# google-deepmind/mujoco_warp

Hardware: NVIDIA H100
Metric: env-steps/sec (whole box) on humanoid.xml at nworld=8192 per GPU (higher is better)
Workload: dtype f32

## Files before the change

### include/mjb200.h

```cpp
#ifndef MJB200_H
#define MJB200_H

#ifdef __cplusplus
extern "C" {
#endif

typedef struct mjbModel mjbModel;
typedef struct mjbData mjbData;

mjbModel* mjb_model_create(void);
void mjb_model_destroy(mjbModel* m);
int mjb_model_set_int(mjbModel* m, const char* name, int value);
int mjb_model_set_float(mjbModel* m, const char* name, float value);
int mjb_model_set_array(mjbModel* m, const char* name, const void* dev_ptr, int nbatch);
int mjb_model_set_array_batched(mjbModel* m, const char* name, const void* dev_ptr, int nbatch, int batch_stride);
int mjb_model_finalize(mjbModel* m);

mjbData* mjb_data_create(int nworld, int nconmax, int naconmax, int njmax, int njmax_pad, int nv_pad);
void mjb_data_destroy(mjbData* d);
int mjb_data_set_array(mjbData* d, const char* name, void* dev_ptr);
int mjb_data_set_int(mjbData* d, const char* name, int value);
int mjb_data_finalize(mjbData* d, const mjbModel* m);

int mjb_step(const mjbModel* m, mjbData* d, void* stream);
// ... 16 lines not shown
int mjb_rne(const mjbModel* m, mjbData* d, void* stream);
int mjb_solve_m(const mjbModel* m, mjbData* d, float* x, const float* y, void* stream);
int mjb_mul_m(const mjbModel* m, mjbData* d, float* res, const float* vec, void* stream);
int mjb_sensor_pos(const mjbModel* m, mjbData* d, void* stream);
int mjb_sensor_vel(const mjbModel* m, mjbData* d, void* stream);
int mjb_sensor_acc(const mjbModel* m, mjbData* d, void* stream);
int mjb_contact_force(const mjbModel* m, mjbData* d, const int* contact_ids, int n, int to_world_frame, float* force, void* stream);
int mjb_rays(const mjbModel* m, mjbData* d, const float* pnt, const float* vec, int nray, int pnt_nbatch, const int* geomgroup,
             int flg_static, const int* bodyexclude, float* dist, int* geomid, float* normal, void* stream);
int mjb_rungekutta4(const mjbModel* m, mjbData* d, void* stream);
int mjb_solve(const mjbModel* m, mjbData* d, void* stream);
int mjb_euler(const mjbModel* m, mjbData* d, void* stream);
int mjb_implicit(const mjbModel* m, mjbData* d, void* stream);
#define MJB_SET_CONST_FIXED 1
#define MJB_SET_CONST_0 2
#define MJB_SET_CONST_SPRING 4
int mjb_set_const(const mjbModel* m, mjbData* d, int parts, int restore, void* stream);
int mjb_ctrl_noise(const mjbModel* m, mjbData* d, const float* ctrl_center, int step, float noise_std, float noise_rate, void* stream);

int mjb_step_profile(const mjbModel* m, mjbData* d, void* stream, float* ms_out);

int mjb_team_residency(const mjbModel* m, const mjbData* d, int* position_worlds, int* velocity_worlds);

int mjb_last_launch_count(void);
const char* mjb_last_error(void);
const char* mjb_version(void);

#ifdef __cplusplus
}
#endif
#endif
```

### mujoco_warp_b200/__init__.py

```python

from . import scenes
from ._src import mjcf
from ._src._lib import build
from ._src.forward import camlight, collision, com_pos, crb, ctrl_noise, euler, factor_m, forward, fwd_acceleration, fwd_actuation
from ._src.forward import fwd_position, fwd_velocity, kinematics, last_launch_count, make_constraint, solve, step, step_profile, team_residency, transmission
from ._src.forward import com_vel, contact_force, fwd_kinematics, get_state, implicit, mul_m, passive, rne, rungekutta4, sensor_acc, sensor_pos, sensor_vel, set_state, solve_m, step1, step2
from ._src.inverse import inverse
from ._src.ray import ray, rays
from ._src.set_const import set_const, set_const_0, set_const_fixed, set_const_spring
from ._src.io import get_data_into, load_trajectory, make_data, override_model, put_data, put_model, reset_data, reset_data_keyframe
from ._src.trace import event_trace_step, flatten_trace
from ._src.types import BroadphaseFilter, BroadphaseType, ConeType, Constraint, ConstraintState, ConstraintType, Contact, Data
from ._src.types import BiasType, DynType, GainType, State, Statistic, TrnType
from ._src.types import DisableBit, EnableBit, GeomType, IntegratorType, JointType, Model, Option, OverflowType, SolverType

__all__ = [n for n in dir() if not n.startswith("_")]
```

### mujoco_warp_b200/_src/forward.py

```python

from __future__ import annotations

import torch

from . import _lib
from .types import Data, Model


def _call(name: str, m: Model, d: Data):
  if d._model is not m and d._model._handle != m._handle:
    raise ValueError("Data was created for a different Model")
  stream = torch.cuda.current_stream().cuda_stream
  _lib.check(getattr(_lib.lib(), name)(m._handle, d._handle, stream))


def step(m: Model, d: Data):
  _call("mjb_step", m, d)


def forward(m: Model, d: Data):
  _call("mjb_forward", m, d)


def fwd_position(m: Model, d: Data):
# ... 202 lines not shown
  return int(_lib.lib().mjb_last_launch_count())


KERNEL_NAMES = ("position", "collision", "constraint", "velocity", "solver", "integrate")


def step_profile(m: Model, d: Data):
  import ctypes

  out = (ctypes.c_float * 6)()
  stream = torch.cuda.current_stream().cuda_stream
  _lib.check(_lib.lib().mjb_step_profile(m._handle, d._handle, stream, out))
  return dict(zip(KERNEL_NAMES, [float(x) for x in out]))


def team_residency(m: Model, d: Data):
  import ctypes

  f = _lib.lib().mjb_team_residency
  f.argtypes = [ctypes.c_void_p, ctypes.c_void_p, ctypes.POINTER(ctypes.c_int), ctypes.POINTER(ctypes.c_int)]
  pos, vel = ctypes.c_int(), ctypes.c_int()
  _lib.check(f(m._handle, d._handle, ctypes.byref(pos), ctypes.byref(vel)))
  return {"position": pos.value, "velocity": vel.value}
```

### mujoco_warp_b200/csrc/capi.cu

```cuda
#include <cstdio>
#include <cstdlib>
#include <algorithm>
#include <cstring>
using std::min;
#include <string>

#include "../../include/mjb200.h"
#include "mjb_launch.cuh"
#include "mjb_types.cuh"

struct mjbModel {
  ModelDev dev;
  FluidDev fluid;
  SensorCollisionDev sc;
  SetConstDev setc;
  bool finalized;
};
struct mjbData {
  DataDev dev;
  bool finalized;
  cudaStream_t aux[8];
  cudaEvent_t ev_fork, ev_join[8];
  int nsplit;
  float* rk;
// ... 165 lines not shown
  if (check(cudaMemset(d->dev.world_ncon, 0, sizeof(int) * (size_t)d->dev.nworld), "memset")) return -1;
  if (check(cudaMalloc(&d->dev.imp_qacc, sizeof(float) * (size_t)d->dev.nworld * (size_t)(m->dev.nv > 0 ? m->dev.nv : 1)), "cudaMalloc(imp_qacc)")) return -1;
  if (!d->inv_qacc && check(cudaMalloc(&d->inv_qacc, sizeof(float) * (size_t)d->dev.nworld * (size_t)(m->dev.nv > 0 ? m->dev.nv : 1)), "cudaMalloc(inv_qacc)")) return -1;
  if (!d->qpos_save && check(cudaMalloc(&d->qpos_save, sizeof(float) * (size_t)d->dev.nworld * (size_t)(m->dev.nq > 0 ? m->dev.nq : 1)), "cudaMalloc(qpos_save)")) return -1;
  if (m->dev.integrator == INT_RK4 && !d->rk &&
      check(cudaMalloc(&d->rk, sizeof(float) * (size_t)d->dev.nworld * (size_t)(m->dev.nq + 3 * m->dev.nv + 2 * m->dev.na + 1)), "cudaMalloc(rk)")) return -1;
  const size_t smem[6] = {smem_position(m->dev, d->dev), smem_collision(m->dev, d->dev), smem_constraint(m->dev, d->dev),
                          smem_velocity(m->dev, d->dev, fluid(m, d)), smem_solver(m->dev, d->dev),    smem_integrate(m->dev)};
  static const char* names[6] = {"position", "collision", "constraint", "velocity", "solver", "integrate"};
  for (int i = 0; i < 6; i++)
    if (smem[i] > kMaxSmem) {
      char buf[160];
      snprintf(buf, sizeof buf, "%s kernel needs %zu B of shared memory per block (> %zu): model/njmax too large for this version", names[i], smem[i], kMaxSmem);
      return fail(buf);
    }
  if (smem_sensor_collision(m->sc) > kMaxSmem) {
    char buf[200];
    snprintf(buf, sizeof buf, "collision-sensor kernel needs %zu B of shared memory per block (> %zu): too many sensor geom pairs or GJK / EPA iterations",
             smem_sensor_collision(m->sc), kMaxSmem);
    return fail(buf);
  }
  {
    const char* e = getenv("MJB_SPLIT");
    const int want = e ? atoi(e) : 2;
    if (want >= 2 && d->dev.nworld >= 1024) {
      const int ns = want > 8 ? 8 : want;
      for (int i = 0; i < ns; i++) {
        if (check(cudaStreamCreateWithFlags(&d->aux[i], cudaStreamNonBlocking), "cudaStreamCreate")) return -1;
        if (check(cudaEventCreateWithFlags(&d->ev_join[i], cudaEventDisableTiming), "cudaEventCreate")) return -1;
      }
      if (check(cudaEventCreateWithFlags(&d->ev_fork, cudaEventDisableTiming), "cudaEventCreate")) return -1;
      d->nsplit = ns;
    }
  }
  d->finalized = true;
  return 0;
}

#define MJB_ENTER()                                                                 \
  if (!m || !d || !m->finalized || !d->finalized) return fail("model/data not finalized"); \
  cudaStream_t s = (cudaStream_t)stream;                                             \
  g_launches = 0;
#define MJB_LAUNCH(call) do { if (check((call), #call)) return -1; } while (0)

int mjb_kinematics(const mjbModel* m, mjbData* d, void* stream) { MJB_ENTER(); MJB_LAUNCH(launch_position(m->dev, d->dev, STG_KINEMATICS, s)); return 0; }
int mjb_com_pos(const mjbModel* m, mjbData* d, void* stream) { MJB_ENTER(); MJB_LAUNCH(launch_position(m->dev, d->dev, STG_COM_POS, s)); return 0; }
int mjb_camlight(const mjbModel* m, mjbData* d, void* stream) { MJB_ENTER(); MJB_LAUNCH(launch_position(m->dev, d->dev, STG_CAMLIGHT, s)); return 0; }
// ... 140 lines not shown
    return rk4_after_forward(m, d, s);
  }
  return pipeline(m, d, RUN_POSITION | RUN_VELOCITY | RUN_SOLVER | RUN_EULER, s);
}
int mjb_step_profile(const mjbModel* m, mjbData* d, void* stream, float* ms_out) {
  MJB_ENTER();
  cudaEvent_t ev[7];
  int n = 0, rc = 0;
  while (n < 7 && !(rc = check(cudaEventCreate(&ev[n]), "cudaEventCreate"))) n++;
  if (!rc) rc = check(reset_contact_counters(d->dev, s), "reset_contact_counters");
  if (!rc) rc = check(cudaEventRecord(ev[0], s), "cudaEventRecord");
  if (!rc) rc = chain(m, d, d->dev, RUN_POSITION | RUN_VELOCITY | RUN_SOLVER | RUN_EULER, s, ev + 1);
  if (!rc) rc = check(cudaEventSynchronize(ev[6]), "cudaEventSynchronize");
  for (int i = 0; i < 6 && !rc; i++) rc = check(cudaEventElapsedTime(&ms_out[i], ev[i], ev[i + 1]), "cudaEventElapsedTime");
  for (int i = 0; i < n; i++) cudaEventDestroy(ev[i]);
  return rc;
}
int mjb_team_residency(const mjbModel* m, const mjbData* d, int* position_worlds, int* velocity_worlds) {
  if (!m || !d || !m->finalized || !d->finalized) return fail("model/data not finalized");
  if (!position_worlds || !velocity_worlds) return fail("mjb_team_residency: null output");
  if (check(resident_worlds_position(m->dev, d->dev, position_worlds), "resident_worlds_position")) return -1;
  if (check(resident_worlds_velocity(m->dev, d->dev, velocity_worlds, fluid(m, d)), "resident_worlds_velocity")) return -1;
  return 0;
}
int mjb_set_const(const mjbModel* m, mjbData* d, int parts, int restore, void* stream) {
  MJB_ENTER();
  if (parts < 1 || parts > (MJB_SET_CONST_FIXED | MJB_SET_CONST_0 | MJB_SET_CONST_SPRING)) return fail("mjb_set_const: parts must be a non-empty combination of MJB_SET_CONST_FIXED / _0 / _SPRING, got " + std::to_string(parts));
  if (restore != 0 && restore != 1) return fail("mjb_set_const: restore must be 0 or 1");
  const ModelDev& md = m->dev;
  const int nworld = d->dev.nworld;
  const bool fixed = parts & MJB_SET_CONST_FIXED, zero = parts & MJB_SET_CONST_0, spring = (parts & MJB_SET_CONST_SPRING) && md.ntendon > 0;
  if (zero && (!m->setc.actuator_acc0 || !m->setc.meaninertia)) return fail("mjb_set_const: model array not set: actuator_acc0 / meaninertia");
  int w_zero = 1, w_spring = md.nb_tendon_lengthspring;
  struct { const char* name; int nb; } out[] = {
    {"body_subtreemass", fixed ? md.nb_body_subtreemass : 1}, {"tendon_lengthspring", spring ? md.nb_tendon_lengthspring : 1},
    {"tendon_length0", md.nb_tendon_length0}, {"eq_data", md.nb_eq_data}, {"dof_invweight0", md.nb_dof_invweight0}, {"body_invweight0", md.nb_body_invweight0},
    {"tendon_invweight0", md.nb_tendon_invweight0}, {"cam_pos0", md.nb_cam_pos0}, {"cam_poscom0", md.nb_cam_poscom0}, {"cam_mat0", md.nb_cam_mat0},
    {"light_pos0", md.nb_light_pos0}, {"light_poscom0", md.nb_light_poscom0}, {"light_dir0", md.nb_light_dir0}, {"actuator_acc0", m->setc.nb_actuator_acc0},
    {"actuator_biasprm", md.nb_actuator_biasprm}};
  for (size_t i = 0; i < sizeof(out) / sizeof(out[0]); i++) {
    const int nb = (i < 2 || zero) ? out[i].nb : 1;
    if (nb > nworld) return fail(std::string("mjb_set_const: Model.") + out[i].name + " has " + std::to_string(nb) + " entries, more than the Data's " + std::to_string(nworld) + " worlds");
    if (i >= 2) w_zero = std::max(w_zero, nb);
  }
  if (zero && smem_set_const(md) > kMaxSmem) {
    char buf[200];
// ... 38 lines not shown
```

### mujoco_warp_b200/csrc/k_solver.cu

```cuda
#include "mjb_chol.cuh"
#include "mjb_launch.cuh"
#include "mjb_linesearch.cuh"
#include "mjb_team.cuh"
#include "mjb_math.cuh"
#include "mjb_types.cuh"

namespace {

struct SolLayout { int J, vec, H, Lf, M, rowf, rowi, ldJ, ldH, nvp, nrowf, cgv, env, bar, total; };
__host__ __device__ inline SolLayout sol_layout(const ModelDev& m, const DataDev& d, bool big) {
  SolLayout L;
  const int cap = d.njmax;
  int o = 0;
  auto take = [&](int n) { int r = o; o += (n + 3) & ~3; return r; };
  L.nvp = d.nv_pad; L.ldJ = d.nv_pad; L.ldH = m.nv | 1;
  L.J = take(big ? 0 : cap * L.ldJ);
  L.vec = take(7 * L.nvp);
  L.cgv = take(m.solver == SOL_CG ? 3 * L.nvp : 0);
  const int hsz = m.nv * (m.nv + 1) / 2;
  L.H = take(hsz);
  L.Lf = take(big ? hsz : cholpair_size(m.nv <= 8 ? 8 : m.nv <= 16 ? 16 : m.nv <= 24 ? 24 : m.nv <= 28 ? 28 : 32));
  L.M = take(big ? m.nC : hsz);
  const bool ell = m.cone == CONE_ELLIPTIC;
  L.nrowf = ((m.nfricdof + m.ntenfric) > 0 ? 5 : 4);
  L.rowf = take((L.nrowf + (ell ? 4 : 0)) * cap);
  L.rowi = take((ell ? 3 : 2) * cap);
  L.env = take(big ? cap + L.nvp : 0);
  L.bar = take(4);
  L.total = o;
  return L;
}

__device__ __forceinline__ P3 warp_sum3(P3 p) { return mkp(warp_sum(p.c), warp_sum(p.g), warp_sum(p.h)); }
__device__ __forceinline__ void tcopy(float* dst, const float* src, int n, int lane) {
#pragma unroll 1
  for (int i = lane; i < n; i += 32) dst[i] = src[i];
}

__device__ __forceinline__ float row_dot(const float* Jr, const float* vec, int nvp) {
  float s = 0.f;
#pragma unroll 4
  for (int k = 0; k < nvp; k += 4) {
    const float4 a = *reinterpret_cast<const float4*>(Jr + k), b = *reinterpret_cast<const float4*>(vec + k);
    s += a.x * b.x + a.y * b.y + a.z * b.z + a.w * b.w;
  }
  return s;
}

struct Ctx {
  const ModelDev* m;
  int lane, nv, nvp, nefc, ne, nf, ldJ, ldH;
  float *J, *H, *Lf, *M, *qacc, *Ma, *grad, *search, *mv, *qfs, *x, *qfc;
  float *Jaref, *jv, *D, *force, *floss, *hw;
  int *state, *hidx;
  float search_dot, grad_dot, newton_decrement, improvement;
  int* rinfo; float *rfri, *quad; int njmax, ncone;
  const float* Jg;
  float* cgv;
  int *rng, *fz;
  bool env;
  float chol_inv;
  int chol_off;
  bool factored;
};
template <bool BIG>
__device__ __forceinline__ const float* jrow(const Ctx& c, int r) {
  if (BIG) return c.Jg + (size_t)r * c.ldJ;
  return c.J + r * c.ldJ;
}
__device__ __forceinline__ EllQ ell_load(const Ctx& c, int r) {
  const float* q = c.quad + 3 * r;
  EllQ e; e.q0 = q[0]; e.q1 = q[1]; e.q2 = q[2]; e.u0 = q[3]; e.v0 = q[4]; e.uu = q[5]; e.uv = q[6]; e.vv = q[7]; e.dm = q[8];
  return e;
}

template <bool BIG>
__device__ __forceinline__ void mul_m(const Ctx& c, const float* vec, float* res) {
  const ModelDev& m = *c.m;
  if (!BIG) {
    const int i = c.lane, nv = c.nv;
    if (i < nv) {
      const float* Mi = c.M + (i * (i + 1)) / 2;
      float acc = 0.f;
      int tk = 0;
#pragma unroll 4
      for (int k = 0; k < nv; k++) {
        const float mk = k <= i ? Mi[k] : c.M[tk + i];
        acc += mk * vec[k];
        tk += k + 1;
      }
      res[i] = acc;
    }
  } else {
#pragma unroll 1
    for (int i = c.lane; i < c.nv; i += 32) {
      float acc = 0.f;
#pragma unroll 4
      for (int k = m.mulm_rowadr[i]; k < m.mulm_rowadr[i + 1]; k++) acc += c.M[m.mulm_madr[k]] * vec[m.mulm_col[k]];
      res[i] = acc;
    }
  }
}

template <bool ELL, bool BIG>
__device__ __forceinline__ int update_constraint(Ctx& c, bool init) {
  int nlist = 0, ncone = 0;
  if (ELL) init = true;
#pragma unroll 1
  for (int r0 = 0; r0 < c.nefc; r0 += 32) {
    const int r = r0 + c.lane;
    bool flip = false, cone0 = false;
    float wgt = 0.f;
    if (r < c.nefc) {
      const float jaref = c.Jaref[r], D = c.D[r];
      const int old = c.state[r];
      float force; int st;
      MJB_ROW_FORCE_STATE(ELL, r, c.ne, c.nf, jaref, D, c.floss, c.rinfo, c.rfri, c.Jaref, c.D, force, st, cone0)
      c.force[r] = force; c.state[r] = st;
      const bool nq = st == ST_QUADRATIC, oq = (!init) && old == ST_QUADRATIC;
      flip = nq != oq;
      wgt = nq ? D : -D;
    }
    const unsigned bal = __ballot_sync(FULL_MASK, flip);
    if (flip) { const int p = nlist + __popc(bal & ((1u << c.lane) - 1u)); c.hidx[p] = r; c.hw[p] = wgt; }
    nlist += __popc(bal);
    if (ELL) {
      const unsigned cb = __ballot_sync(FULL_MASK, cone0);
      if (cone0) c.hidx[c.njmax - 1 - (ncone + __popc(cb & ((1u << c.lane) - 1u)))] = r;
      ncone += __popc(cb);
    }
  }
  c.ncone = ncone;
  __syncwarp();
#pragma unroll 1
  for (int dd = c.lane; dd < c.nv; dd += 32) {
    float s = 0.f;
#pragma unroll 8
    for (int r = 0; r < c.nefc; r++) s += jrow<BIG>(c, r)[dd] * c.force[r];
    c.qfc[dd] = s;
  }
  __syncwarp();
  return nlist;
}

__device__ __forceinline__ void update_grad(Ctx& c) {
  float gd = 0.f;
#pragma unroll 1
  for (int dd = c.lane; dd < c.nv; dd += 32) { const float g = c.Ma[dd] - c.qfs[dd] - c.qfc[dd]; c.grad[dd] = g; gd += g * g; }
  c.grad_dot = warp_sum(gd);
  __syncwarp();
}

struct ConeK { float dm, mu, mu_tinv, munttt, tdiag; int dim; };
__device__ __forceinline__ ConeK cone_scalars(const Ctx& c, int e0) {
  ConeK k;
  k.dim = c.rinfo[e0] >> 4; k.mu = c.rfri[e0];
  const float mu2 = k.mu * k.mu;
  k.dm = safe_div(c.D[e0], mu2 * (1.0f + mu2));
  const float n = c.Jaref[e0] * k.mu;
  float tt = 0.f;
  for (int j = 1; j < k.dim; j++) { const float u = c.Jaref[e0 + j] * c.rfri[e0 + j]; tt += u * u; }
  const float t = fmaxf(sqrtf(tt), MJ_MINVAL), ttt = fmaxf(t * t * t, MJ_MINVAL);
  k.mu_tinv = safe_div(k.mu, t); k.munttt = k.mu * safe_div(n, ttt); k.tdiag = mu2 - n * k.mu_tinv;
  return k;
}
__device__ __forceinline__ float cone_coef(const Ctx& c, const ConeK& k, int e0, int j, float J0i, float pi, float Jji) {
  if (j == 0) return k.dm * k.mu * (k.mu * J0i - k.mu_tinv * pi);
  const float s = c.rfri[e0 + j], us = c.Jaref[e0 + j] * s * s;
  return k.dm * ((k.munttt * pi - k.mu_tinv * k.mu * J0i) * us + k.tdiag * s * s * Jji);
}

// ... 31 lines not shown
      float pi = 0.f;
      for (int j = 1; j < k.dim; j++) pi += c.Jaref[e0 + j] * c.rfri[e0 + j] * c.rfri[e0 + j] * (lane < nv ? J0[j * c.ldJ + lane] : 0.f);
#pragma unroll 1
      for (int j = 0; j < k.dim; j++) {
        const float* Jr = J0 + j * c.ldJ;
        const float sc = lane < nv ? cone_coef(c, k, e0, j, J0i, pi, Jr[lane]) : 0.f;
#pragma unroll
        for (int q = 0; q < N; q += 4) {
          const float4 v = *reinterpret_cast<const float4*>(Jr + q);
          a[q] += sc * v.x; a[q + 1] += sc * v.y; a[q + 2] += sc * v.z; a[q + 3] += sc * v.w;
        }
      }
    }
  }
  c.factored = true;
  return chol_solve_rows_pair<N>(a, nv, g, c.Lf, lane, c.chol_inv, c.chol_off);
}

template <bool ELL, bool BIG, int NREG = 0>
__device__ __forceinline__ void update_search(Ctx& c, int nlist) {
  const int nv = c.nv;
  float sd = 0.f, nd = 0.f;
  if (!BIG) {
    const float g = c.lane < nv ? c.grad[c.lane] : 0.f;
    float xx;
    if (!ELL && nlist == 0 && c.factored) xx = chol_subst_pair(nv, g, c.Lf, c.lane, c.chol_inv, c.chol_off);
    else if (NREG == 28) xx = newton_direction_reg<28, ELL>(c, nlist, g);
    else if (NREG == 32) xx = newton_direction_reg<32, ELL>(c, nlist, g);
    else if (nv <= 8) xx = newton_direction_reg<8, ELL>(c, nlist, g);
    else if (nv <= 16) xx = newton_direction_reg<16, ELL>(c, nlist, g);
    else if (nv <= 24) xx = newton_direction_reg<24, ELL>(c, nlist, g);
    else if (nv <= 28) xx = newton_direction_reg<28, ELL>(c, nlist, g);
    else xx = newton_direction_reg<32, ELL>(c, nlist, g);
    sd = xx * xx; nd = g * xx;
    if (c.lane < nv) c.search[c.lane] = -xx;
  } else {
    const int ntri = nv * (nv + 1) / 2;
    float* Hd = ELL ? c.Lf : c.H;
    if (ELL) {
#pragma unroll 1
      for (int e = c.lane; e < ntri; e += 32) c.Lf[e] = c.H[e];
      __syncwarp();
    }
#pragma unroll 1
    for (int t = 0; t < nlist; t++) {
      const float* Jr = jrow<true>(c, c.hidx[t]);
      const float wt = c.hw[t];
// ... 42 lines not shown
    } else {
      warp_cholesky_packed(c.Lf, nv, c.lane);
      warp_chol_solve_packed(c.Lf, nv, c.x, c.lane);
    }
#pragma unroll 1
    for (int dd = c.lane; dd < nv; dd += 32) { const float xx = c.x[dd]; sd += xx * xx; nd += c.grad[dd] * xx; c.search[dd] = -xx; }
  }
  c.search_dot = warp_sum(sd); c.newton_decrement = warp_sum(nd);
  __syncwarp();
}

template <bool ELL>
__device__ __forceinline__ P3 eval_total(const Ctx& c, float alpha, float q0, float q1, float q2) {
  P3 s = mkp(0.f, 0.f, 0.f);
#pragma unroll 1
  for (int r = c.lane; r < c.nefc; r += 32) {
    if (ELL && c.rinfo[r] != -1) {
      if (c.rinfo[r] >= 0 && (c.rinfo[r] & 15) == 0) { const EllQ q = ell_load(c, r); const float mu = c.rfri[r]; s = s + ell_shifted(mu, q, ell_reference(mu, q), alpha); }
    } else s = s + eval_row(r, alpha, c.ne, c.nf, c.D[r], c.floss[r], c.Jaref[r], c.jv[r]);
  }
  return eval_gauss(q0, q1, q2, alpha) + warp_sum3(s);
}

template <bool ELL, bool BIG>
__device__ __forceinline__ bool linesearch(Ctx& c) {
  const ModelDev& m = *c.m;
  const int nv = c.nv;
  mul_m<BIG>(c, c.search, c.mv);
#pragma unroll 1
  for (int r = c.lane; r < c.nefc; r += 32) {
    c.jv[r] = row_dot(jrow<BIG>(c, r), c.search, c.nvp);
  }
  __syncwarp();
  const float snorm = sqrtf(c.search_dot), scale = m.meaninertia * (float)nv;
  const float gtol = fmaxf(m.tolerance * m.ls_tolerance * snorm * scale, 1e-6f);
  P3 p0s = mkp(0.f, 0.f, 0.f);
  if (ELL) {
#pragma unroll 1
    for (int r = c.lane; r < c.nefc; r += 32) {
      const int info = c.rinfo[r];
      if (info < 0 || (info & 15) != 0) continue;
      const int dim = info >> 4;
      const float mu = c.rfri[r], ja = c.Jaref[r], jv = c.jv[r], D = c.D[r], jvD = jv * D;
      float q0 = 0.5f * ja * ja * D, q1 = jvD * ja, q2 = 0.5f * jv * jvD, uu = 0.f, uv = 0.f, vv = 0.f;
      for (int j = 1; j < dim; j++) {
        const float jvj = c.jv[r + j], jaj = c.Jaref[r + j], dj = c.D[r + j], DJ = dj * jaj, fj = c.rfri[r + j];
        q0 += 0.5f * jaj * DJ; q1 += jvj * DJ; q2 += 0.5f * jvj * dj * jvj;
        const float uj = jaj * fj, vj = jvj * fj;
        uu += uj * uj; uv += uj * vj; vv += vj * vj;
      }
      float* q = c.quad + 3 * r;
      const float mu2 = mu * mu;
      q[0] = q0; q[1] = q1; q[2] = q2; q[3] = ja * mu; q[4] = jv * mu; q[5] = uu; q[6] = uv; q[7] = vv; q[8] = D / (mu2 * (1.0f + mu2));
    }
    __syncwarp();
  }
#pragma unroll 1
  for (int r = c.lane; r < c.nefc; r += 32) {
    if (ELL && c.rinfo[r] != -1) {
      if (c.rinfo[r] >= 0 && (c.rinfo[r] & 15) == 0) p0s = p0s + ell_zero(c.rfri[r], ell_load(c, r));
    } else p0s = p0s + eval_row_zero(r, c.ne, c.nf, c.D[r], c.floss[r], c.Jaref[r], c.jv[r]);
  }
  float g1 = 0.f, g2 = 0.f;
#pragma unroll 1
  for (int dd = c.lane; dd < nv; dd += 32) { const float s = c.search[dd]; g1 += s * (c.Ma[dd] - c.qfs[dd]); g2 += 0.5f * s * c.mv[dd]; }
  p0s = warp_sum3(p0s);
  const float q0 = 0.f, q1 = warp_sum(g1), q2 = warp_sum(g2);
  const P3 p0 = mkp(q0 + p0s.c, q1 + p0s.g, 2.0f * q2 + p0s.h);
  const P3 p0_delta = mkp(0.f, p0.g, p0.h);
  const float lo_alpha_in = -safe_div(p0.g, p0.h);
  const P3 lo_in = eval_total<ELL>(c, lo_alpha_in, q0, q1, q2);
  const bool initial_converged = fabsf(lo_in.g) < gtol && lo_in.c < 0.f;
  bool ls_converged = initial_converged;
  float alpha = 0.f, improvement = 0.f;
  if (!initial_converged) {
    const bool lo_less = lo_in.g < p0.g;
    P3 lo = lo_less ? lo_in : p0_delta, hi = lo_less ? p0_delta : lo_in;
    float lo_alpha = lo_less ? lo_alpha_in : 0.f, hi_alpha = lo_less ? 0.f : lo_alpha_in;
#pragma unroll 1
    for (int it = 0; it < m.ls_iterations; it++) {
      const float lo_next_alpha = lo_alpha - safe_div(lo.g, lo.h), hi_next_alpha = hi_alpha - safe_div(hi.g, hi.h), mid_alpha = 0.5f * (lo_alpha + hi_alpha);
      P3 sl = mkp(0.f, 0.f, 0.f), sh = sl, sm = sl;
#pragma unroll 1
      for (int r = c.lane; r < c.nefc; r += 32) {
        if (ELL && c.rinfo[r] != -1) {
          if (c.rinfo[r] >= 0 && (c.rinfo[r] & 15) == 0) {
            const EllQ q = ell_load(c, r); const float mu = c.rfri[r]; const EllRef e = ell_reference(mu, q);
            sl = sl + ell_shifted(mu, q, e, lo_next_alpha); sh = sh + ell_shifted(mu, q, e, hi_next_alpha); sm = sm + ell_shifted(mu, q, e, mid_alpha);
// ... 3 lines not shown
        const float D = c.D[r], f = c.floss[r], ja = c.Jaref[r], jv = c.jv[r];
        sl = sl + eval_row(r, lo_next_alpha, c.ne, c.nf, D, f, ja, jv);
        sh = sh + eval_row(r, hi_next_alpha, c.ne, c.nf, D, f, ja, jv);
        sm = sm + eval_row(r, mid_alpha, c.ne, c.nf, D, f, ja, jv);
      }
      const P3 lo_next = eval_gauss(q0, q1, q2, lo_next_alpha) + warp_sum3(sl);
      const P3 hi_next = eval_gauss(q0, q1, q2, hi_next_alpha) + warp_sum3(sh);
      const P3 mid = eval_gauss(q0, q1, q2, mid_alpha) + warp_sum3(sm);
      const bool s1 = in_bracket(lo, lo_next); if (s1) { lo = lo_next; lo_alpha = lo_next_alpha; }
      const bool s2 = in_bracket(lo, mid); if (s2) { lo = mid; lo_alpha = mid_alpha; }
      const bool s3 = in_bracket(lo, hi_next); if (s3) { lo = hi_next; lo_alpha = hi_next_alpha; }
      const bool h1 = in_bracket(hi, hi_next); if (h1) { hi = hi_next; hi_alpha = hi_next_alpha; }
      const bool h2 = in_bracket(hi, mid); if (h2) { hi = mid; hi_alpha = mid_alpha; }
      const bool h3 = in_bracket(hi, lo_next); if (h3) { hi = lo_next; hi_alpha = lo_next_alpha; }
      const bool swap_lo = s1 || s2 || s3, swap_hi = h1 || h2 || h3;
      const bool ls_done = (!swap_lo && !swap_hi) || (lo.c < 0.f && lo.g < 0.f && lo.g > -gtol) || (hi.c < 0.f && hi.g > 0.f && hi.g < gtol);
      const bool improved = lo.c < 0.f || hi.c < 0.f, lo_better = lo.c < hi.c;
      if (improved) { alpha = lo_better ? lo_alpha : hi_alpha; improvement = -(lo_better ? lo.c : hi.c); }
      if (ls_done) { ls_converged = true; break; }
    }
  } else {
    alpha = lo_alpha_in; improvement = -lo_in.c;
  }
#pragma unroll 1
  for (int dd = c.lane; dd < nv; dd += 32) { c.qacc[dd] += alpha * c.search[dd]; c.Ma[dd] += alpha * c.mv[dd]; }
#pragma unroll 1
  for (int r = c.lane; r < c.nefc; r += 32) c.Jaref[r] += alpha * c.jv[r];
  c.improvement = improvement;
  __syncwarp();
  return ls_converged;
}

__device__ __forceinline__ void cg_direction(Ctx& c, const ModelDev& m, const DataDev& d, size_t wb, bool init) {
  const int nv = c.nv, lane = c.lane;
  float *Mg = c.cgv, *pg = c.cgv + c.nvp, *pMg = c.cgv + 2 * c.nvp;
#pragma unroll 1
  for (int dd = lane; dd < nv; dd += 32) Mg[dd] = c.grad[dd];
  __syncwarp();
#pragma unroll 1
  for (int t = 0; t < m.ntree; t++) {
    const int start = m.tree_dofadr[t], n = m.tree_dofnum[t];
    const float* U = d.qLD + wb * m.qld_total + m.tree_qLDadr[t];
    float* xt = Mg + start;
#pragma unroll 1
    for (int j = 0; j < n; j++) {
      const float zj = xt[j] / U[j * n + j];
      __syncwarp();
      for (int i = j + 1 + lane; i < n; i += 32) xt[i] -= U[j * n + i] * zj;
// ... 10 lines not shown
    }
  }
  float beta = 0.f;
  if (!init) {
    float num = 0.f, den = 0.f;
#pragma unroll 1
    for (int dd = lane; dd < nv; dd += 32) { num += c.grad[dd] * (Mg[dd] - pMg[dd]); den += pg[dd] * pMg[dd]; }
    beta = fmaxf(0.f, warp_sum(num) / fmaxf(MJ_MINVAL, warp_sum(den)));
  }
  float sd = 0.f;
#pragma unroll 1
  for (int dd = lane; dd < nv; dd += 32) {
    const float sv = -Mg[dd] + beta * c.search[dd];
    c.search[dd] = sv; sd += sv * sv;
    pg[dd] = c.grad[dd]; pMg[dd] = Mg[dd];
  }
  c.search_dot = warp_sum(sd);
  __syncwarp();
}

template <bool ELL, bool BIG, bool CG, bool PLAIN = false, int NREG = 0>
__global__ void __launch_bounds__(32, BIG ? 1 : 16)
k_solver(const __grid_constant__ ModelDev m, const __grid_constant__ DataDev d) {
  extern __shared__ float smem[];
  const int lane = threadIdx.x;
  const int w = blockIdx.x + d.w0;
  if (w >= d.nworld) return;
  const SolLayout L = sol_layout(m, d, BIG);
  float* S = smem;
  const int nv = m.nv, njmax = d.njmax, nvp = d.nv_pad;
  const size_t wb = (size_t)w;
  Ctx c;
  c.factored = false; c.chol_inv = 1.0f; c.chol_off = 0;
  c.m = &m; c.lane = lane; c.nv = nv; c.nvp = L.nvp; c.ldJ = L.ldJ; c.ldH = L.ldH;
  if (NREG > 0) { c.nvp = NREG; c.ldJ = NREG; }
  c.J = S + L.J; c.H = S + L.H; c.Lf = S + L.Lf; c.M = S + L.M;
  float* v = S + L.vec;
  const int vp = L.nvp;
  c.qacc = v; c.Ma = v + vp; c.grad = v + 2 * vp; c.search = v + 3 * vp; c.mv = v + 4 * vp; c.x = c.mv; c.qfs = v + 5 * vp; c.qfc = v + 6 * vp;
  float* rf = S + L.rowf;
  c.Jaref = rf; c.jv = rf + njmax; c.hw = c.jv; c.D = rf + 2 * njmax; c.force = rf + 3 * njmax;
  c.floss = (m.nfricdof + m.ntenfric) > 0 ? rf + 4 * njmax : c.D;
  int* ri = (int*)(S + L.rowi);
  c.state = ri; c.hidx = ri + njmax;
  c.njmax = njmax; c.ncone = 0;
  c.Jg = d.efc_J + wb * (size_t)d.njmax_pad * nvp;
  c.cgv = S + L.cgv;
  c.rng = (int*)(S + L.env); c.fz = c.rng + njmax;
  c.env = BIG && m.ntree > 1;
  c.rfri = rf + L.nrowf * njmax; c.quad = c.rfri + njmax; c.rinfo = ri + 2 * njmax;

  if (njmax == 0 || nv == 0) {
#pragma unroll 1
    for (int dd = lane; dd < nv; dd += 32) d.qacc[wb * nv + dd] = d.qacc_smooth[wb * nv + dd];
    if (lane == 0) d.solver_niter[w] = 0;
    return;
  }
  const int nefc = min(d.nefc[w], njmax);
  c.nefc = nefc; c.ne = PLAIN ? 0 : d.ne[w]; c.nf = PLAIN ? 0 : d.nf[w];

  Stager st;
  const int n4 = (nefc + 3) & ~3, nrow = n4 <= njmax ? n4 : nefc;
  st.init(reinterpret_cast<uint64_t*>(S + L.bar), lane);
  if (!BIG) st.load(c.J, c.Jg, nefc * nvp);
  st.load(c.D, d.efc_D + wb * d.njmax_pad, nrow);
  st.load(c.Jaref, d.efc_aref + wb * njmax, nrow);
  if ((m.nfricdof + m.ntenfric) > 0) st.load(c.floss, d.efc_frictionloss + wb * njmax, nrow);
  for (int i = lane; i < 7 * vp; i += 32) v[i] = 0.f;
  __syncwarp();
#pragma unroll 1
  for (int r = lane; r < nefc; r += 32) {
    c.state[r] = ST_SATISFIED;
    if (ELL) {
      int info = -1; float fr = 0.f;
      if (d.efc_type[wb * njmax + r] == CNSTR_CONTACT_ELLIPTIC) {
        const int cid = d.efc_id[wb * njmax + r], e0 = d.contact_efc_address[(size_t)cid * m.nmaxpyramid], dim = d.contact_dim[cid], j = r - e0;
        info = (e0 < 0 || e0 + dim > nefc) ? -2 : ((dim << 4) | j);
        fr = j == 0 ? d.contact_friction[5 * (size_t)cid] * m.impratio_invsqrt : d.contact_friction[5 * (size_t)cid + j - 1];
      }
      c.rinfo[r] = info; c.rfri[r] = fr;
    }
  }
  if (BIG) tcopy(c.M, d.M + wb * m.nC, m.nC, lane);
  tcopy(c.qfs, d.qfrc_smooth + wb * nv, nv, lane);
  const float* start = (m.disableflags & DSBL_WARMSTART) ? d.qacc_smooth : d.qacc_warmstart;
  tcopy(c.qacc, start + wb * nv, nv, lane);
  const int hsz = nv * (nv + 1) / 2;
#pragma unroll 1
  for (int e = lane; e < hsz; e += 32) { c.H[e] = 0.f; if (!BIG) c.M[e] = 0.f; }
  __syncwarp();
  if (c.env) {
#pragma unroll 1
    for (int i = lane; i < nv; i += 32) c.fz[i] = i;
    __syncwarp();
  }
  if (!BIG) {
    const float* Mg = d.M + wb * m.nC;
#pragma unroll 4
    for (int e = lane; e < m.nC; e += 32) {
      const int r = m.M_entry_row[e], col = m.M_colind[e];
      const float v = Mg[e];
      c.M[(r * (r + 1)) / 2 + col] = v;
      c.H[(r * (r + 1)) / 2 + col] = v;
    }
  } else {
#pragma unroll 1
    for (int e = lane; e < m.nC; e += 32) {
// ... 16 lines not shown
    if (ELL) {
#pragma unroll 1
      for (int r = lane; r < nefc; r += 32) {
        const int info = c.rinfo[r];
        if (info < 0 || (info & 15) != 0) continue;
        const int dim = info >> 4;
        int lo = nv, hi = 0;
        for (int j = 0; j < dim; j++) { const int g = c.rng[r + j]; if ((g >> 16) > 0) { lo = min(lo, g & 0xFFFF); hi = max(hi, g >> 16); } }
        if (hi == 0) lo = 0;
        for (int j = 0; j < dim; j++) c.rng[r + j] = lo | (hi << 16);
      }
      __syncwarp();
    }
#pragma unroll 1
    for (int r = lane; r < nefc; r += 32) {
      const int lo = c.rng[r] & 0xFFFF, hi = c.rng[r] >> 16;
      for (int i = lo; i < hi; i++) atomicMin(&c.fz[i], lo);
    }
  }
#pragma unroll 1
  for (int r = lane; r < nefc; r += 32) {
    c.Jaref[r] = row_dot(jrow<BIG>(c, r), c.qacc, c.nvp) - c.Jaref[r];
  }
  mul_m<BIG>(c, c.qacc, c.Ma);
  __syncwarp();

  const float scale = m.meaninertia * (float)nv;
  int niter = 0, ovf = 0;
  for (int it = -1;; it++) {
    if (it >= 0 && !linesearch<ELL, BIG>(c)) ovf |= OVF_LS_ITERATIONS;
    const int nlist = update_constraint<ELL, BIG>(c, it < 0);
    update_grad(c);
    if (it >= 0) {
      niter++;
      const float improvement = c.improvement / scale, gradient = sqrtf(c.grad_dot) / scale;
      if (improvement < m.tolerance || gradient < m.tolerance) break;
    } else if (m.iterations == 0) break;
    if (CG) {
      if (it >= 0 && niter == m.iterations) { ovf |= OVF_ITERATIONS; break; }
      cg_direction(c, m, d, wb, it < 0);
      continue;
    }
    if (!CG) update_search<ELL, BIG, NREG>(c, nlist);
    if (it >= 0) {
      if (0.5f * c.newton_decrement / scale < m.tolerance) break;
      if (niter == m.iterations) { ovf |= OVF_ITERATIONS; break; }
    }
  }

  tcopy(d.qacc + wb * nv, c.qacc, nv, lane);
  tcopy(d.efc_Ma + wb * nv, c.Ma, nv, lane);
  tcopy(d.qfrc_constraint + wb * nv, c.qfc, nv, lane);
#pragma unroll 1
  for (int r = lane; r < nefc; r += 32) { d.efc_force[wb * njmax + r] = c.force[r]; d.efc_state[wb * d.njmax_pad + r] = c.state[r]; }
  if (lane == 0) { d.solver_niter[w] = niter; if (ovf) d.overflow[w] |= ovf; }
}

}

size_t smem_solver(const ModelDev& m, const DataDev& d) { return (size_t)sol_layout(m, d, m.nv > 32).total * sizeof(float); }

cudaError_t launch_solver(const ModelDev& m, const DataDev& d, cudaStream_t s) {
  const int ell = m.cone == CONE_ELLIPTIC ? 1 : 0, big = m.nv > 32 ? 1 : 0, cg = m.solver == SOL_CG ? 1 : 0;
  const int which = 4 * cg + 2 * big + ell;
  static void (*const kerns[8])(ModelDev, DataDev) = {
    k_solver<false, false, false>, k_solver<true, false, false>, k_solver<false, true, false>, k_solver<true, true, false>,
    k_solver<false, false, true>,  k_solver<true, false, true>,  k_solver<false, true, true>,  k_solver<true, true, true>};
  void (*kern)(ModelDev, DataDev) = kerns[which];
  const bool plain = m.neq == 0 && m.nfricdof == 0 && m.ntenfric == 0 && m.ntendon == 0;
  if (which == 0 && plain) {
    kern = k_solver<false, false, false, true>;
    if (m.nv > 24 && m.nv <= 28 && d.nv_pad == 28) kern = k_solver<false, false, false, true, 28>;
    else if (m.nv > 28 && d.nv_pad == 32) kern = k_solver<false, false, false, true, 32>;
  }
  if (which == 2 && plain) kern = k_solver<false, true, false, true>;
  return launch(kern, d.wn, 32, smem_solver(m, d), s, m, d);
}
```

### mujoco_warp_b200/csrc/mjb_types.cuh

```cuda
#pragma once
#include <cuda_runtime.h>

#define MJB_MODEL_INTS(X) \
  X(nq) X(nv) X(nu) X(nbody) X(njnt) X(ngeom) X(nsite) X(ncam) X(nlight) X(nC) X(ntree) X(nJmom) X(nlevel) \
  X(nxn_npair) X(nlimit) X(nfricdof) X(nmaxpyramid) X(integrator) X(cone) X(solver) X(iterations) \
  X(ls_iterations) X(disableflags) X(enableflags) X(broadphase) X(broadphase_filter) X(qld_total) X(maxtree) X(has_multicontact_geom) X(neq) X(nlimit_ball) X(has_gravcomp) X(nmocap) X(npair) X(has_convex_pair) X(ccd_iterations) X(epa_iterations) X(nsensor) X(nsensordata) X(sensor_subtree_vel) X(sensor_rne_postconstraint) X(nmesh) X(na) X(ntendon) X(nJten) X(ntenfric) X(nwrap) X(nmat) X(nmeshface)
#define MJB_MODEL_FLOATS(X) \
  X(timestep) X(tolerance) X(ls_tolerance) X(impratio_invsqrt) X(meaninertia) X(gravity_x) X(gravity_y) X(gravity_z) X(ccd_tolerance)
#define MJB_MODEL_IARRS(X) \
  X(body_parentid) X(body_rootid) X(body_weldid) X(body_mocapid) X(body_jntnum) X(body_jntadr) X(body_dofnum) X(body_dofadr) \
  X(body_childadr) X(body_childid) X(level_adr) X(level_body) \
  X(jnt_type) X(jnt_qposadr) X(jnt_dofadr) X(jnt_bodyid) X(jnt_actfrclimited) X(jnt_actgravcomp) X(jnt_limited_adr) \
  X(dof_bodyid) X(dof_jntid) X(dof_parentid) X(dof_fricloss_adr) X(M_rownnz) X(M_rowadr) X(M_colind) X(M_entry_row) X(mulm_rowadr) X(mulm_col) X(mulm_madr) \
  X(tree_dofadr) X(tree_dofnum) X(tree_qLDadr) \
  X(geom_type) X(geom_condim) X(geom_bodyid) X(geom_priority) \
  X(actuator_trnid) X(actuator_gaintype) X(actuator_biastype) X(actuator_ctrllimited) X(actuator_forcelimited) \
  X(actuator_dyntype) X(actuator_actadr) X(actuator_actnum) X(actuator_actlimited) X(actuator_actearly) X(actuator_trntype) \
  X(ten_J_rownnz) X(ten_J_rowadr) X(ten_J_colind) X(tendon_adr) X(tendon_num) X(wrap_objid) X(tendon_limited) X(tendon_actfrclimited) \
  X(moment_rownnz0) X(moment_rowadr0) X(moment_colind0) X(dofact_adr) X(dofact_act) X(dofact_mom) \
  X(cam_mode) X(cam_bodyid) X(cam_targetbodyid) X(light_mode) X(light_bodyid) X(light_targetbodyid) X(site_bodyid) \
  X(nxn_geom_pair) X(nxn_pairid) X(body_isdofancestor) X(eq_type) X(eq_obj1id) X(eq_obj2id) X(jnt_limited_ball_adr) X(pair_dim) \
  X(sensor_type) X(sensor_datatype) X(sensor_needstage) X(sensor_objtype) X(sensor_objid) X(sensor_reftype) X(sensor_refid) X(sensor_dim) X(sensor_adr) X(site_type) \
  X(geom_dataid) X(mesh_vertadr) X(mesh_vertnum) X(mesh_graphadr) X(mesh_graph) X(mesh_polynum) X(mesh_polyadr) X(mesh_polyvertadr) X(mesh_polyvertnum) \
  X(mesh_polyvert) X(mesh_polymapadr) X(mesh_polymapnum) X(mesh_polymap) X(geom_group) X(geom_matid) X(mesh_faceadr) X(mesh_face)
// ... 158 lines not shown
cudaError_t launch_velocity(const ModelDev& m, const DataDev& d, int stage_mask, cudaStream_t s, const FluidDev& f);
cudaError_t launch_solve_m(const ModelDev& m, const DataDev& d, float* x, const float* y, cudaStream_t s);
cudaError_t launch_mul_m(const ModelDev& m, const DataDev& d, float* res, const float* vec, cudaStream_t s);
cudaError_t launch_solver(const ModelDev& m, const DataDev& d, cudaStream_t s);
cudaError_t launch_integrate(const ModelDev& m, const DataDev& d, int integrator, cudaStream_t s, const FluidDev& f);
cudaError_t launch_implicit_solve(const ModelDev& m, const DataDev& d, float* qacc_out, cudaStream_t s);
size_t smem_implicit(const ModelDev& m);
cudaError_t launch_sensor(const ModelDev& m, const DataDev& d, int stages, cudaStream_t s, const SensorCollisionDev& c);
cudaError_t launch_sensor_collision(const ModelDev& m, const DataDev& d, const SensorCollisionDev& c, cudaStream_t s);
size_t smem_sensor_collision(const SensorCollisionDev& c);
cudaError_t launch_contact_force(const ModelDev& m, const DataDev& d, const int* contact_ids, int n, int to_world, float* out, cudaStream_t s);
cudaError_t launch_inverse(const ModelDev& m, const DataDev& d, float* qfrc_inverse, float* qacc_cont, bool disc, cudaStream_t s, const FluidDev& f);
cudaError_t launch_rk_stage(const ModelDev& m, const DataDev& d, float* rk, int stage, cudaStream_t s);
cudaError_t launch_ray(const ModelDev& m, const DataDev& d, const float* pnt, const float* vec, int nray, int pnt_nbatch, const int* geomgroup, int flg_static,
                       const int* bodyexclude, float* dist, int* geomid, float* normal, cudaStream_t s);
cudaError_t launch_ctrl_noise(const ModelDev& m, const DataDev& d, const float* ctrl_center, int step, float std, float rate, cudaStream_t s);
size_t smem_position(const ModelDev& m, const DataDev& d);
size_t smem_collision(const ModelDev& m, const DataDev& d);
size_t smem_constraint(const ModelDev& m, const DataDev& d);
size_t smem_velocity(const ModelDev& m, const DataDev& d, const FluidDev& f);
cudaError_t resident_worlds_position(const ModelDev& m, const DataDev& d, int* worlds);
cudaError_t resident_worlds_velocity(const ModelDev& m, const DataDev& d, int* worlds, const FluidDev& f);
size_t smem_solver(const ModelDev& m, const DataDev& d);
cudaError_t launch_set_const_fixed(const ModelDev& m, int nw, int nworld, cudaStream_t s);
cudaError_t launch_set_const_qpos(const ModelDev& m, const DataDev& d, const SetConstDev& c, int mode, int nw, cudaStream_t s);
cudaError_t launch_set_const_0(const ModelDev& m, const DataDev& d, const SetConstDev& c, int nw, cudaStream_t s);
cudaError_t launch_set_const_spring(const ModelDev& m, const DataDev& d, int nw, cudaStream_t s);
size_t smem_set_const(const ModelDev& m);
size_t smem_integrate(const ModelDev& m);
```

Baseline: 20.65 million.

## Shrink solver shared memory: register-resident vectors and narrow state/hidx types

```diff
diff --git a/include/mjb200.h b/include/mjb200.h
--- a/include/mjb200.h
+++ b/include/mjb200.h
@@ -62,6 +62,9 @@
 
 int mjb_team_residency(const mjbModel* m, const mjbData* d, int* position_worlds, int* velocity_worlds);
 
+int mjb_solver_residency(const mjbModel* m, const mjbData* d, int* worlds, int* registers, int* smem_bytes);
+int mjb_solver_smem(const mjbModel* m, const mjbData* d);
+
 int mjb_last_launch_count(void);
 const char* mjb_last_error(void);
 const char* mjb_version(void);
diff --git a/mujoco_warp_b200/__init__.py b/mujoco_warp_b200/__init__.py
--- a/mujoco_warp_b200/__init__.py
+++ b/mujoco_warp_b200/__init__.py
@@ -3,7 +3,7 @@
 from ._src import mjcf
 from ._src._lib import build
 from ._src.forward import camlight, collision, com_pos, crb, ctrl_noise, euler, factor_m, forward, fwd_acceleration, fwd_actuation
-from ._src.forward import fwd_position, fwd_velocity, kinematics, last_launch_count, make_constraint, solve, step, step_profile, team_residency, transmission
+from ._src.forward import fwd_position, fwd_velocity, kinematics, last_launch_count, make_constraint, solve, solver_residency, step, step_profile, team_residency, transmission
 from ._src.forward import com_vel, contact_force, fwd_kinematics, get_state, implicit, mul_m, passive, rne, rungekutta4, sensor_acc, sensor_pos, sensor_vel, set_state, solve_m, step1, step2
 from ._src.inverse import inverse
 from ._src.ray import ray, rays
diff --git a/mujoco_warp_b200/_src/forward.py b/mujoco_warp_b200/_src/forward.py
--- a/mujoco_warp_b200/_src/forward.py
+++ b/mujoco_warp_b200/_src/forward.py
@@ -248,3 +248,13 @@
   pos, vel = ctypes.c_int(), ctypes.c_int()
   _lib.check(f(m._handle, d._handle, ctypes.byref(pos), ctypes.byref(vel)))
   return {"position": pos.value, "velocity": vel.value}
+
+
+def solver_residency(m: Model, d: Data):
+  import ctypes
+
+  f = _lib.lib().mjb_solver_residency
+  f.argtypes = [ctypes.c_void_p, ctypes.c_void_p] + [ctypes.POINTER(ctypes.c_int)] * 3
+  worlds, regs, smem = ctypes.c_int(), ctypes.c_int(), ctypes.c_int()
+  _lib.check(f(m._handle, d._handle, ctypes.byref(worlds), ctypes.byref(regs), ctypes.byref(smem)))
+  return {"worlds": worlds.value, "registers": regs.value, "smem_bytes": smem.value}
diff --git a/mujoco_warp_b200/csrc/capi.cu b/mujoco_warp_b200/csrc/capi.cu
--- a/mujoco_warp_b200/csrc/capi.cu
+++ b/mujoco_warp_b200/csrc/capi.cu
@@ -211,7 +211,7 @@
   }
   {
     const char* e = getenv("MJB_SPLIT");
-    const int want = e ? atoi(e) : 2;
+    const int want = e ? atoi(e) : std::min(4, std::max(2, d->dev.nworld / 2048));
     if (want >= 2 && d->dev.nworld >= 1024) {
       const int ns = want > 8 ? 8 : want;
       for (int i = 0; i < ns; i++) {
@@ -398,6 +398,16 @@
   if (check(resident_worlds_position(m->dev, d->dev, position_worlds), "resident_worlds_position")) return -1;
   if (check(resident_worlds_velocity(m->dev, d->dev, velocity_worlds, fluid(m, d)), "resident_worlds_velocity")) return -1;
   return 0;
+}
+int mjb_solver_residency(const mjbModel* m, const mjbData* d, int* worlds, int* registers, int* smem_bytes) {
+  if (!m || !d || !m->finalized || !d->finalized) return fail("model/data not finalized");
+  if (!worlds || !registers || !smem_bytes) return fail("mjb_solver_residency: null output");
+  *smem_bytes = (int)smem_solver(m->dev, d->dev);
+  return check(resident_worlds_solver(m->dev, d->dev, worlds, registers), "resident_worlds_solver");
+}
+int mjb_solver_smem(const mjbModel* m, const mjbData* d) {
+  if (!m || !d) return fail("mjb_solver_smem: null model or data");
+  return (int)smem_solver(m->dev, d->dev);
 }
 int mjb_set_const(const mjbModel* m, mjbData* d, int parts, int restore, void* stream) {
   MJB_ENTER();
diff --git a/mujoco_warp_b200/csrc/k_solver.cu b/mujoco_warp_b200/csrc/k_solver.cu
--- a/mujoco_warp_b200/csrc/k_solver.cu
+++ b/mujoco_warp_b200/csrc/k_solver.cu
@@ -7,7 +7,7 @@
 
 namespace {
 
-struct SolLayout { int J, vec, H, Lf, M, rowf, rowi, ldJ, ldH, nvp, nrowf, cgv, env, bar, total; };
+struct SolLayout { int J, vec, nvec, H, Lf, M, rowf, state, hidx, rinfo, ldJ, ldH, nvp, nrowf, cgv, env, bar, total; };
 __host__ __device__ inline SolLayout sol_layout(const ModelDev& m, const DataDev& d, bool big) {
   SolLayout L;
   const int cap = d.njmax;
@@ -15,7 +15,8 @@
   auto take = [&](int n) { int r = o; o += (n + 3) & ~3; return r; };
   L.nvp = d.nv_pad; L.ldJ = d.nv_pad; L.ldH = m.nv | 1;
   L.J = take(big ? 0 : cap * L.ldJ);
-  L.vec = take(7 * L.nvp);
+  L.nvec = (big || m.solver == SOL_CG) ? 7 : 3;
+  L.vec = take(L.nvec * L.nvp);
   L.cgv = take(m.solver == SOL_CG ? 3 * L.nvp : 0);
   const int hsz = m.nv * (m.nv + 1) / 2;
   L.H = take(hsz);
@@ -24,7 +25,9 @@
   const bool ell = m.cone == CONE_ELLIPTIC;
   L.nrowf = ((m.nfricdof + m.ntenfric) > 0 ? 5 : 4);
   L.rowf = take((L.nrowf + (ell ? 4 : 0)) * cap);
-  L.rowi = take((ell ? 3 : 2) * cap);
+  L.state = take((cap + 3) / 4);
+  L.hidx = take((cap + 1) / 2);
+  L.rinfo = take(ell ? cap : 0);
   L.env = take(big ? cap + L.nvp : 0);
   L.bar = take(4);
   L.total = o;
@@ -51,8 +54,10 @@
   const ModelDev* m;
   int lane, nv, nvp, nefc, ne, nf, ldJ, ldH;
   float *J, *H, *Lf, *M, *qacc, *Ma, *grad, *search, *mv, *qfs, *x, *qfc;
+  float Ma_i, grad_i, qfs_i, qfc_i;
   float *Jaref, *jv, *D, *force, *floss, *hw;
-  int *state, *hidx;
+  uint8_t* state;
+  uint16_t* hidx;
   float search_dot, grad_dot, newton_decrement, improvement;
   int* rinfo; float *rfri, *quad; int njmax, ncone;
   const float* Jg;
@@ -74,23 +79,27 @@
   return e;
 }
 
+__device__ __forceinline__ float mul_m_lane(const Ctx& c, const float* vec) {
+  const int i = c.lane, nv = c.nv;
+  float acc = 0.f;
+  if (i < nv) {
+    const float* Mi = c.M + (i * (i + 1)) / 2;
+    int tk = 0;
+#pragma unroll 4
+    for (int k = 0; k < nv; k++) {
+      const float mk = k <= i ? Mi[k] : c.M[tk + i];
+      acc += mk * vec[k];
+      tk += k + 1;
+    }
+  }
+  return acc;
+}
 template <bool BIG>
 __device__ __forceinline__ void mul_m(const Ctx& c, const float* vec, float* res) {
   const ModelDev& m = *c.m;
   if (!BIG) {
-    const int i = c.lane, nv = c.nv;
-    if (i < nv) {
-      const float* Mi = c.M + (i * (i + 1)) / 2;
-      float acc = 0.f;
-      int tk = 0;
-#pragma unroll 4
-      for (int k = 0; k < nv; k++) {
-        const float mk = k <= i ? Mi[k] : c.M[tk + i];
-        acc += mk * vec[k];
-        tk += k + 1;
-      }
-      res[i] = acc;
-    }
+    const float acc = mul_m_lane(c, vec);
+    if (c.lane < c.nv) res[c.lane] = acc;
   } else {
 #pragma unroll 1
     for (int i = c.lane; i < c.nv; i += 32) {
@@ -102,7 +111,7 @@
   }
 }
 
-template <bool ELL, bool BIG>
+template <bool ELL, bool BIG, bool REGV>
 __device__ __forceinline__ int update_constraint(Ctx& c, bool init) {
   int nlist = 0, ncone = 0;
   if (ELL) init = true;
@@ -132,21 +141,35 @@
   }
   c.ncone = ncone;
   __syncwarp();
-#pragma unroll 1
-  for (int dd = c.lane; dd < c.nv; dd += 32) {
-    float s = 0.f;
+  if (REGV) {
+    if (c.lane < c.nv) {
+      float s = 0.f;
 #pragma unroll 8
-    for (int r = 0; r < c.nefc; r++) s += jrow<BIG>(c, r)[dd] * c.force[r];
-    c.qfc[dd] = s;
-  }
-  __syncwarp();
+      for (int r = 0; r < c.nefc; r++) s += jrow<BIG>(c, r)[c.lane] * c.force[r];
+      c.qfc_i = s;
+    }
+  } else {
+#pragma unroll 1
+    for (int dd = c.lane; dd < c.nv; dd += 32) {
+      float s = 0.f;
+#pragma unroll 8
+      for (int r = 0; r < c.nefc; r++) s += jrow<BIG>(c, r)[dd] * c.force[r];
+      c.qfc[dd] = s;
+    }
+    __syncwarp();
+  }
   return nlist;
 }
 
+template <bool REGV>
 __device__ __forceinline__ void update_grad(Ctx& c) {
   float gd = 0.f;
-#pragma unroll 1
-  for (int dd = c.lane; dd < c.nv; dd += 32) { const float g = c.Ma[dd] - c.qfs[dd] - c.qfc[dd]; c.grad[dd] = g; gd += g * g; }
+  if (REGV) {
+    if (c.lane < c.nv) { const float g = c.Ma_i - c.qfs_i - c.qfc_i; c.grad_i = g; gd += g * g; }
+  } else {
+#pragma unroll 1
+    for (int dd = c.lane; dd < c.nv; dd += 32) { const float g = c.Ma[dd] - c.qfs[dd] - c.qfc[dd]; c.grad[dd] = g; gd += g * g; }
+  }
   c.grad_dot = warp_sum(gd);
   __syncwarp();
 }
@@ -224,7 +247,7 @@
   const int nv = c.nv;
   float sd = 0.f, nd = 0.f;
   if (!BIG) {
-    const float g = c.lane < nv ? c.grad[c.lane] : 0.f;
+    const float g = c.lane < nv ? c.grad_i : 0.f;
     float xx;
     if (!ELL && nlist == 0 && c.factored) xx = chol_subst_pair(nv, g, c.Lf, c.lane, c.chol_inv, c.chol_off);
     else if (NREG == 28) xx = newton_direction_reg<28, ELL>(c, nlist, g);
@@ -313,7 +336,7 @@
   return eval_gauss(q0, q1, q2, alpha) + warp_sum3(s);
 }
 
-template <bool ELL, bool BIG>
+template <bool ELL, bool BIG, bool REGV>
 __device__ __forceinline__ bool linesearch(Ctx& c) {
   const ModelDev& m = *c.m;
   const int nv = c.nv;
@@ -353,8 +376,12 @@
     } else p0s = p0s + eval_row_zero(r, c.ne, c.nf, c.D[r], c.floss[r], c.Jaref[r], c.jv[r]);
   }
   float g1 = 0.f, g2 = 0.f;
-#pragma unroll 1
-  for (int dd = c.lane; dd < nv; dd += 32) { const float s = c.search[dd]; g1 += s * (c.Ma[dd] - c.qfs[dd]); g2 += 0.5f * s * c.mv[dd]; }
+  if (REGV) {
+    if (c.lane < nv) { const float s = c.search[c.lane]; g1 += s * (c.Ma_i - c.qfs_i); g2 += 0.5f * s * c.mv[c.lane]; }
+  } else {
+#pragma unroll 1
+    for (int dd = c.lane; dd < nv; dd += 32) { const float s = c.search[dd]; g1 += s * (c.Ma[dd] - c.qfs[dd]); g2 += 0.5f * s * c.mv[dd]; }
+  }
   p0s = warp_sum3(p0s);
   const float q0 = 0.f, q1 = warp_sum(g1), q2 = warp_sum(g2);
   const P3 p0 = mkp(q0 + p0s.c, q1 + p0s.g, 2.0f * q2 + p0s.h);
@@ -404,8 +431,12 @@
   } else {
     alpha = lo_alpha_in; improvement = -lo_in.c;
   }
-#pragma unroll 1
-  for (int dd = c.lane; dd < nv; dd += 32) { c.qacc[dd] += alpha * c.search[dd]; c.Ma[dd] += alpha * c.mv[dd]; }
+  if (REGV) {
+    if (c.lane < nv) { c.qacc[c.lane] += alpha * c.search[c.lane]; c.Ma_i += alpha * c.mv[c.lane]; }
+  } else {
+#pragma unroll 1
+    for (int dd = c.lane; dd < nv; dd += 32) { c.qacc[dd] += alpha * c.search[dd]; c.Ma[dd] += alpha * c.mv[dd]; }
+  }
 #pragma unroll 1
   for (int r = c.lane; r < c.nefc; r += 32) c.Jaref[r] += alpha * c.jv[r];
   c.improvement = improvement;
@@ -462,6 +493,7 @@
 template <bool ELL, bool BIG, bool CG, bool PLAIN = false, int NREG = 0>
 __global__ void __launch_bounds__(32, BIG ? 1 : 16)
 k_solver(const __grid_constant__ ModelDev m, const __grid_constant__ DataDev d) {
+  constexpr bool REGV = !BIG && !CG;
   extern __shared__ float smem[];
   const int lane = threadIdx.x;
   const int w = blockIdx.x + d.w0;
@@ -477,18 +509,23 @@
   c.J = S + L.J; c.H = S + L.H; c.Lf = S + L.Lf; c.M = S + L.M;
   float* v = S + L.vec;
   const int vp = L.nvp;
-  c.qacc = v; c.Ma = v + vp; c.grad = v + 2 * vp; c.search = v + 3 * vp; c.mv = v + 4 * vp; c.x = c.mv; c.qfs = v + 5 * vp; c.qfc = v + 6 * vp;
+  c.Ma_i = 0.f; c.grad_i = 0.f; c.qfs_i = 0.f; c.qfc_i = 0.f;
+  if (REGV) {
+    c.qacc = v; c.search = v + vp; c.mv = v + 2 * vp; c.x = c.mv;
+    c.Ma = c.grad = c.qfs = c.qfc = nullptr;
+  } else {
+    c.qacc = v; c.Ma = v + vp; c.grad = v + 2 * vp; c.search = v + 3 * vp; c.mv = v + 4 * vp; c.x = c.mv; c.qfs = v + 5 * vp; c.qfc = v + 6 * vp;
+  }
   float* rf = S + L.rowf;
   c.Jaref = rf; c.jv = rf + njmax; c.hw = c.jv; c.D = rf + 2 * njmax; c.force = rf + 3 * njmax;
   c.floss = (m.nfricdof + m.ntenfric) > 0 ? rf + 4 * njmax : c.D;
-  int* ri = (int*)(S + L.rowi);
-  c.state = ri; c.hidx = ri + njmax;
+  c.state = reinterpret_cast<uint8_t*>(S + L.state); c.hidx = reinterpret_cast<uint16_t*>(S + L.hidx);
   c.njmax = njmax; c.ncone = 0;
   c.Jg = d.efc_J + wb * (size_t)d.njmax_pad * nvp;
   c.cgv = S + L.cgv;
   c.rng = (int*)(S + L.env); c.fz = c.rng + njmax;
   c.env = BIG && m.ntree > 1;
-  c.rfri = rf + L.nrowf * njmax; c.quad = c.rfri + njmax; c.rinfo = ri + 2 * njmax;
+  c.rfri = rf + L.nrowf * njmax; c.quad = c.rfri + njmax; c.rinfo = (int*)(S + L.rinfo);
 
   if (njmax == 0 || nv == 0) {
 #pragma unroll 1
@@ -506,7 +543,7 @@
   st.load(c.D, d.efc_D + wb * d.njmax_pad, nrow);
   st.load(c.Jaref, d.efc_aref + wb * njmax, nrow);
   if ((m.nfricdof + m.ntenfric) > 0) st.load(c.floss, d.efc_frictionloss + wb * njmax, nrow);
-  for (int i = lane; i < 7 * vp; i += 32) v[i] = 0.f;
+  for (int i = lane; i < L.nvec * vp; i += 32) v[i] = 0.f;
   __syncwarp();
 #pragma unroll 1
   for (int r = lane; r < nefc; r += 32) {
@@ -522,7 +559,8 @@
     }
   }
   if (BIG) tcopy(c.M, d.M + wb * m.nC, m.nC, lane);
-  tcopy(c.qfs, d.qfrc_smooth + wb * nv, nv, lane);
+  if (REGV) c.qfs_i = lane < nv ? d.qfrc_smooth[wb * nv + lane] : 0.f;
+  else tcopy(c.qfs, d.qfrc_smooth + wb * nv, nv, lane);
   const float* start = (m.disableflags & DSBL_WARMSTART) ? d.qacc_smooth : d.qacc_warmstart;
   tcopy(c.qacc, start + wb * nv, nv, lane);
   const int hsz = nv * (nv + 1) / 2;
@@ -585,15 +623,16 @@
   for (int r = lane; r < nefc; r += 32) {
     c.Jaref[r] = row_dot(jrow<BIG>(c, r), c.qacc, c.nvp) - c.Jaref[r];
   }
-  mul_m<BIG>(c, c.qacc, c.Ma);
+  if (REGV) c.Ma_i = mul_m_lane(c, c.qacc);
+  else mul_m<BIG>(c, c.qacc, c.Ma);
   __syncwarp();
 
   const float scale = m.meaninertia * (float)nv;
   int niter = 0, ovf = 0;
   for (int it = -1;; it++) {
-    if (it >= 0 && !linesearch<ELL, BIG>(c)) ovf |= OVF_LS_ITERATIONS;
-    const int nlist = update_constraint<ELL, BIG>(c, it < 0);
-    update_grad(c);
+    if (it >= 0 && !linesearch<ELL, BIG, REGV>(c)) ovf |= OVF_LS_ITERATIONS;
+    const int nlist = update_constraint<ELL, BIG, REGV>(c, it < 0);
+    update_grad<REGV>(c);
     if (it >= 0) {
       niter++;
       const float improvement = c.improvement / scale, gradient = sqrtf(c.grad_dot) / scale;
@@ -612,8 +651,12 @@
   }
 
   tcopy(d.qacc + wb * nv, c.qacc, nv, lane);
-  tcopy(d.efc_Ma + wb * nv, c.Ma, nv, lane);
-  tcopy(d.qfrc_constraint + wb * nv, c.qfc, nv, lane);
+  if (REGV) {
+    if (lane < nv) { d.efc_Ma[wb * nv + lane] = c.Ma_i; d.qfrc_constraint[wb * nv + lane] = c.qfc_i; }
+  } else {
+    tcopy(d.efc_Ma + wb * nv, c.Ma, nv, lane);
+    tcopy(d.qfrc_constraint + wb * nv, c.qfc, nv, lane);
+  }
 #pragma unroll 1
   for (int r = lane; r < nefc; r += 32) { d.efc_force[wb * njmax + r] = c.force[r]; d.efc_state[wb * d.njmax_pad + r] = c.state[r]; }
   if (lane == 0) { d.solver_niter[w] = niter; if (ovf) d.overflow[w] |= ovf; }
@@ -623,7 +666,8 @@
 
 size_t smem_solver(const ModelDev& m, const DataDev& d) { return (size_t)sol_layout(m, d, m.nv > 32).total * sizeof(float); }
 
-cudaError_t launch_solver(const ModelDev& m, const DataDev& d, cudaStream_t s) {
+using SolverKernel = void (*)(ModelDev, DataDev);
+static SolverKernel solver_kernel(const ModelDev& m, const DataDev& d) {
   const int ell = m.cone == CONE_ELLIPTIC ? 1 : 0, big = m.nv > 32 ? 1 : 0, cg = m.solver == SOL_CG ? 1 : 0;
   const int which = 4 * cg + 2 * big + ell;
   static void (*const kerns[8])(ModelDev, DataDev) = {
@@ -637,5 +681,17 @@
     else if (m.nv > 28 && d.nv_pad == 32) kern = k_solver<false, false, false, true, 32>;
   }
   if (which == 2 && plain) kern = k_solver<false, true, false, true>;
-  return launch(kern, d.wn, 32, smem_solver(m, d), s, m, d);
-}
+  return kern;
+}
+
+cudaError_t launch_solver(const ModelDev& m, const DataDev& d, cudaStream_t s) { return launch(solver_kernel(m, d), d.wn, 32, smem_solver(m, d), s, m, d); }
+
+cudaError_t resident_worlds_solver(const ModelDev& m, const DataDev& d, int* worlds, int* regs) {
+  const SolverKernel kern = solver_kernel(m, d);
+  const size_t bytes = smem_solver(m, d);
+  *worlds = 0;
+  *regs = kernel_regs(kern);
+  cudaError_t e = launch_configure((const void*)kern, bytes);
+  if (e == cudaSuccess) e = cudaOccupancyMaxActiveBlocksPerMultiprocessor(worlds, kern, 32, bytes);
+  return e;
+}
diff --git a/mujoco_warp_b200/csrc/mjb_types.cuh b/mujoco_warp_b200/csrc/mjb_types.cuh
--- a/mujoco_warp_b200/csrc/mjb_types.cuh
+++ b/mujoco_warp_b200/csrc/mjb_types.cuh
@@ -204,6 +204,7 @@
 cudaError_t resident_worlds_position(const ModelDev& m, const DataDev& d, int* worlds);
 cudaError_t resident_worlds_velocity(const ModelDev& m, const DataDev& d, int* worlds, const FluidDev& f);
 size_t smem_solver(const ModelDev& m, const DataDev& d);
+cudaError_t resident_worlds_solver(const ModelDev& m, const DataDev& d, int* worlds, int* regs);
 cudaError_t launch_set_const_fixed(const ModelDev& m, int nw, int nworld, cudaStream_t s);
 cudaError_t launch_set_const_qpos(const ModelDev& m, const DataDev& d, const SetConstDev& c, int mode, int nw, cudaStream_t s);
 cudaError_t launch_set_const_0(const ModelDev& m, const DataDev& d, const SetConstDev& c, int nw, cudaStream_t s);
```

Measured after the change: 21.20 million, median of 6. 1.03x the previous value.
